# sarpel/wakeword-jupyterlab

Measured on AMD Instinct MI355X. Metric: 1s/16kHz clips/sec end-to-end (mel+CNN+LSTM), higher is better.
Workload: dtype f32 in/out/accumulate; conv and LSTM-gate GEMM products as f16x3 split (3 f16 MFMAs per fp32 product block, ~2^-21 rel.)

## Files before the change

### wakeword-jupyterlab_amd/csrc/ww_logmel.hip

```cpp
#include <mutex>
#include <type_traits>

#include "ww_internal.h"

namespace ww {

constexpr int kSlab = 2048 + 4;
constexpr int kPartialInSlab = 1032;
static_assert(kPartialInSlab + kPieces <= kSlab, "piece sums must fit behind the power spectrum");

template <int WAVES, int FR = kFrames>
struct K1Layout {
    static constexpr int kWaves = WAVES;
    static constexpr int kThreads = WAVES * 64;
    static constexpr int kMelStr = FR + 1;
    static constexpr int kOffMel = WAVES * kSlab;
    static constexpr int kOffRed = kOffMel + kMels * kMelStr;
    static constexpr int kOffFrm = kOffRed + 16;
    static constexpr int kOffInvw = kOffFrm + WAVES * FR;
    static constexpr int kOffFlag = kOffInvw + kMels;
    static constexpr int kOffDcNy = kOffFlag + 4;
    static constexpr int kOffPinfo = kOffDcNy + FR;
    static constexpr int kOffFp0 = kOffPinfo + kPieces;
    static constexpr int kOffFcnt = kOffFp0 + kMels;
    static constexpr int kOffTw2 = kOffFcnt + kMels;
    static constexpr int kOffTwp = kOffTw2 + 7 * 16 * 2;
    static constexpr int kLdsFloats = kOffTwp + 512 * 2;
    static constexpr int kWavesPerSimd = WAVES == 4 ? (FR != kFrames ? 2 : 3) : 2;
    static constexpr int kBlocksPerCu = WAVES == 4 ? (FR != kFrames ? 2 : 3) : 1;
    static_assert(kOffPinfo % 4 == 0 && kOffTw2 % 4 == 0 && kOffTwp % 2 == 0, "LDS table alignment");
    static_assert(FR % WAVES == 0 && WAVES <= 8, "frames are dealt to the waves in whole rounds; red[] holds 16 floats");
    static_assert(FR == kFrames || FR == 64, "the long-clip tile: 64 frames, frames dealt round-robin");
    static_assert(kBlocksPerCu * sizeof(float) * kLdsFloats <= 160 * 1024, "LDS per CU");
};

__device__ __forceinline__ float2 operator+(float2 a, float2 b) { return make_float2(a.x + b.x, a.y + b.y); }
__device__ __forceinline__ float2 operator-(float2 a, float2 b) { return make_float2(a.x - b.x, a.y - b.y); }
__device__ __forceinline__ float2 cmul(float2 a, float2 b) {
    return make_float2(fmaf(a.x, b.x, -a.y * b.y), fmaf(a.x, b.y, a.y * b.x));
}
__device__ __forceinline__ float2 mul_neg_i(float2 a) { return make_float2(a.y, -a.x); }

__device__ __forceinline__ void dft4(float2& a0, float2& a1, float2& a2, float2& a3) {
    const float2 t0 = a0 + a2, t1 = a0 - a2, t2 = a1 + a3, t3 = mul_neg_i(a1 - a3);
    a0 = t0 + t2; a2 = t0 - t2; a1 = t1 + t3; a3 = t1 - t3;
}

__device__ __forceinline__ void dft8(float2 (&v)[8]) {
    constexpr float c = 0.70710678118654752440f;
    float2 e0 = v[0], e1 = v[2], e2 = v[4], e3 = v[6];
    float2 o0 = v[1], o1 = v[3], o2 = v[5], o3 = v[7];
    dft4(e0, e1, e2, e3);
    dft4(o0, o1, o2, o3);
    o1 = make_float2(c * (o1.x + o1.y), c * (o1.y - o1.x));
    o2 = mul_neg_i(o2);
    o3 = make_float2(c * (o3.y - o3.x), -c * (o3.x + o3.y));
    v[0] = e0 + o0; v[4] = e0 - o0;
    v[1] = e1 + o1; v[5] = e1 - o1;
    v[2] = e2 + o2; v[6] = e2 - o2;
    v[3] = e3 + o3; v[7] = e3 - o3;
}

__device__ __forceinline__ void dft16(float2 (&v)[16]) {
    float2 e[8], o[8];
#pragma unroll
    for (int i = 0; i < 8; ++i) { e[i] = v[2 * i]; o[i] = v[2 * i + 1]; }
    dft8(e);
    dft8(o);
    constexpr float c1 = 0.92387953251128675613f, s1 = 0.38268343236508977173f;
    constexpr float c2 = 0.70710678118654752440f;
    const float2 w[8] = {{1.f, 0.f}, {c1, -s1}, {c2, -c2}, {s1, -c1}, {0.f, -1.f}, {-s1, -c1}, {-c2, -c2}, {-c1, -s1}};
#pragma unroll
    for (int k = 0; k < 8; ++k) {
        const float2 t = (k == 0) ? o[0] : (k == 4 ? mul_neg_i(o[4]) : cmul(o[k], w[k]));
        v[k] = e[k] + t;
        v[k + 8] = e[k] - t;
    }
}

__device__ __forceinline__ float db10(float x) {
#pragma clang fp contract(off)
    return 10.0f * log10f(x);
}

__device__ __forceinline__ void lds_order() {
    __builtin_amdgcn_fence(__ATOMIC_RELEASE, "wavefront");
    __builtin_amdgcn_wave_barrier();
    __builtin_amdgcn_fence(__ATOMIC_ACQUIRE, "wavefront");
}

__device__ __forceinline__ float absmax3(float a, float b, float m) {
    float r;
    asm("v_max3_f32 %0, |%1|, |%2|, %3" : "=v"(r) : "v"(a), "v"(b), "v"(m));
    return r;
}

using u32x4_t = __attribute__((ext_vector_type(4))) unsigned int;

template <bool RING>
__device__ __forceinline__ void load_frame(float4 (&sn)[8], __amdgpu_buffer_rsrc_t rsrc, int base, int ring_pos, int ring_len) {
#pragma unroll
    for (int n1 = 0; n1 < 8; ++n1) {
        const int idx = base + 256 * n1;
        int off = idx * 4;
        if constexpr (RING) {
            int at = idx + ring_pos;
            at = at >= ring_len ? at - ring_len : at;
            off = (idx >= 0 && idx < ring_len) ? at * 4 : -1;
        }
        const u32x4_t v = __builtin_amdgcn_raw_buffer_load_b128(rsrc, off, 0, 0);
        sn[n1] = __builtin_bit_cast(float4, v);
    }
}

constexpr uint32_t kRedoMark = 0x7fc5a11eu;
constexpr float kFloorRatio = 1.0e-5f;

#ifdef WW_STAMPS
__device__ unsigned long long g_stamps[16];
#define STAMP(i) do { unsigned long long t__; asm volatile("s_memtime %0\n\ts_waitcnt lgkmcnt(0)" : "=s"(t__) :: "memory"); \
    if (stamp_on) { acc_st[i] += t__ - last_st; } last_st = t__; } while (0)
#else
#define STAMP(i) do {} while (0)
#endif

template <bool RING, int WAVES, int FR = kFrames>
__global__ __launch_bounds__(WAVES * 64, (K1Layout<WAVES, FR>::kWavesPerSimd)) void logmel_kernel(const float* __restrict__ pcm, int64_t clip_stride,
                                                             int clip_len, int n_clips, int normalize,
                                                             const int32_t* __restrict__ ring_pos_p, int ring_len,
                                                             const LogmelTables* __restrict__ tb,
                                                             float* __restrict__ out, int mark, int n_frames) {
    using L = K1Layout<WAVES, FR>;
    constexpr int kMelStride = L::kMelStr;
    const int nfr = FR == kFrames ? kFrames : n_frames;
    constexpr int kWavesPerBlock = WAVES, kThreads = L::kThreads;
    constexpr int kOffMel = L::kOffMel, kOffRed = L::kOffRed, kOffFrm = L::kOffFrm, kOffInvw = L::kOffInvw, kOffFlag = L::kOffFlag,
                  kOffDcNy = L::kOffDcNy, kOffPinfo = L::kOffPinfo, kOffFp0 = L::kOffFp0,
                  kOffFcnt = L::kOffFcnt, kOffTw2 = L::kOffTw2, kOffTwp = L::kOffTwp;
    extern __shared__ __attribute__((aligned(16))) float lds[];
    float* mel = lds + kOffMel;
    float* red = lds + kOffRed;
    const float4* pw4 = reinterpret_cast<const float4*>(&tb->piece_w[0][0][0]);
    const int* pinfo = reinterpret_cast<const int*>(lds + kOffPinfo);
    const int* fp0 = reinterpret_cast<const int*>(lds + kOffFp0);
    const int* fcnt = reinterpret_cast<const int*>(lds + kOffFcnt);
    const float4* tw2_4 = reinterpret_cast<const float4*>(lds + kOffTw2);
    const float2* twp_2 = reinterpret_cast<const float2*>(lds + kOffTwp);

    const int tid = threadIdx.x;
    const int lane_id = tid & 63;
    const int lane = lane_id;
    const int wave = __builtin_amdgcn_readfirstlane(tid >> 6);
    float* slab = lds + wave * kSlab;
    float2* slab2 = reinterpret_cast<float2*>(slab);
    float4* slab4 = reinterpret_cast<float4*>(slab);
    float* partial = slab + kPartialInSlab;
    const float4* tw1_4 = reinterpret_cast<const float4*>(&tb->tw1[0][0]);
    const float4* win4 = reinterpret_cast<const float4*>(&tb->window[0]);

    for (int i = tid; i < kPieces; i += kThreads) reinterpret_cast<int*>(lds)[kOffPinfo + i] = tb->piece_info[i];
    if (tid < kMels) {
        reinterpret_cast<int*>(lds)[kOffFp0 + tid] = tb->filt_p0[tid];
        reinterpret_cast<int*>(lds)[kOffFcnt + tid] = tb->filt_cnt[tid];
        lds[kOffInvw + tid] = tb->band_bins[tid];
    }
    if (tid < 4) reinterpret_cast<uint32_t*>(lds)[kOffFlag + tid] = 0u;
    for (int i = tid; i < 7 * 16 * 2; i += kThreads) lds[kOffTw2 + i] = (&tb->tw2[0][0].x)[i];
    for (int i = tid; i < 512 * 2; i += kThreads) lds[kOffTwp + i] = (&tb->twp[0].x)[i];
    const int ring_pos = RING ? *ring_pos_p : 0;
    __syncthreads();
    const int my_p0a = fp0[lane], my_cnta = fcnt[lane];
    const int my_p0b = lane + 64 < kMels ? fp0[lane + 64] : 0, my_cntb = lane + 64 < kMels ? fcnt[lane + 64] : 0;

#ifdef WW_STAMPS
    const bool stamp_on = true;
    unsigned long long acc_st[10] = {0, 0, 0, 0, 0, 0, 0, 0, 0, 0}, last_st = 0;
    STAMP(9);
#endif

    const unsigned clip_bytes = unsigned(clip_len) * 4u;
    auto clip_rsrc = [&](int c) {
        const bool ok = c < n_clips;
        const float* base = pcm + int64_t(ok ? c : 0) * clip_stride;
        return __builtin_amdgcn_make_buffer_rsrc(const_cast<float*>(base), 0, ok ? clip_bytes : 0u, 0x00020000);
    };
    const int kRounds = FR == kFrames ? kFrames / kWavesPerBlock : (nfr + kWavesPerBlock - 1) / kWavesPerBlock;
    const int frame0 = wave;
    float4 sn[8];
    load_frame<RING>(sn, clip_rsrc(blockIdx.x), frame0 * kHop - kNfft / 2 + 4 * lane, ring_pos, ring_len);
    int clip_it = 0;
#pragma unroll 1
    for (int clip = blockIdx.x; clip < n_clips; clip += gridDim.x, ++clip_it) {
        const __amdgpu_buffer_rsrc_t rs_cur = clip_rsrc(clip), rs_next = clip_rsrc(clip + int(gridDim.x));
        float peak = 0.f;

#pragma unroll 1
        for (int round = 0; round < kRounds; ++round) {
            const int frame = round * kWavesPerBlock + wave;
            int lane = lane_id;
            asm volatile("" : "+v"(lane));
            const int k1r = lane >> 3, jr = lane & 7;
            const int base_next = (frame + kWavesPerBlock) * kHop - kNfft / 2 + 4 * lane;

            STAMP(8);
            float2 za[8], zb[8];
#pragma unroll
            for (int n1 = 0; n1 < 8; ++n1) {
                const float4 s = sn[n1];
                const float4 w = win4[64 * n1 + lane];
                if (n1 == 4 || n1 == 5) peak = absmax3(s.z, s.w, absmax3(s.x, s.y, peak));
                za[n1] = make_float2(s.x * w.x, s.y * w.y);
                zb[n1] = make_float2(s.z * w.z, s.w * w.w);
            }
            float4 t1[7];
#pragma unroll
            for (int k1 = 1; k1 < 8; ++k1) t1[k1 - 1] = tw1_4[(k1 - 1) * 64 + lane];
            __builtin_amdgcn_sched_barrier(0);
            dft8(za);
            dft8(zb);
            slab4[lane] = make_float4(za[0].x, za[0].y, zb[0].x, zb[0].y);
#pragma unroll
            for (int k1 = 1; k1 < 8; ++k1) {
                const float4 t = t1[k1 - 1];
                const float2 a = cmul(za[k1], make_float2(t.x, t.y));
                const float2 b = cmul(zb[k1], make_float2(t.z, t.w));
                slab4[k1 * 64 + (lane ^ (8 * ((k1 >> 1) & 1)))] = make_float4(a.x, a.y, b.x, b.y);
            }
            lds_order();
            STAMP(0);
            {
                const int s8 = 8 * ((k1r >> 1) & 1);
                const float4* x1e = slab4 + k1r * 64 + jr + s8;
                const float4* x1o = slab4 + k1r * 64 + jr - s8;
#pragma unroll
                for (int n2 = 0; n2 < 8; ++n2) {
                    const float4 v = (n2 & 1) ? x1o[n2 * 8] : x1e[n2 * 8];
                    za[n2] = make_float2(v.x, v.y);
                    zb[n2] = make_float2(v.z, v.w);
                }
                float4 t2[7];
#pragma unroll
                for (int k2 = 1; k2 < 8; ++k2) t2[k2 - 1] = tw2_4[(k2 - 1) * 8 + jr];
                lds_order();
                __builtin_amdgcn_sched_barrier(0);
                dft8(za);
                dft8(zb);
                float4* x2w[4];
#pragma unroll
                for (int hk = 0; hk < 4; ++hk) x2w[hk] = slab4 + 64 * k1r + (jr ^ (4 * (k1r & 1) + hk));
#pragma unroll
                for (int k2 = 0; k2 < 8; ++k2) {
                    float2 a = za[k2], b = zb[k2];
                    if (k2 > 0) {
                        const float4 t = t2[k2 - 1];
                        a = cmul(a, make_float2(t.x, t.y));
                        b = cmul(b, make_float2(t.z, t.w));
                    }
                    x2w[k2 >> 1][8 * k2] = make_float4(a.x, a.y, b.x, b.y);
                }
            }
            lds_order();
            STAMP(1);
            {
                float2 u[16];
                const int sw2 = (lane >> 1) & 7;
#pragma unroll
                for (int m = 0; m < 8; ++m) {
                    const float4 v = slab4[lane * 8 + (m ^ sw2)];
                    u[2 * m] = make_float2(v.x, v.y);
                    u[2 * m + 1] = make_float2(v.z, v.w);
                }
                lds_order();
                dft16(u);
                const int lp = (lane >> 3) + 8 * (lane & 7);
                float2* zw = slab2 + (lp ^ (((lp >> 4) & 3) << 1));
#pragma unroll
                for (int kk = 0; kk < 16; ++kk) zw[64 * kk] = u[kk];
            }
            lds_order();
            STAMP(2);
            float4 pw0[kPieceRounds], pw1[kPieceRounds];
#pragma unroll
            for (int c = 0; c < kPieceRounds; ++c) {
                pw0[c] = pw4[c * kPieceSlots + lane];
                pw1[c] = pw4[kPieces + c * kPieceSlots + lane];
            }
            {
                const bool last = round + 1 == kRounds;
                load_frame<RING>(sn, last ? rs_next : rs_cur, last ? frame0 * kHop - kNfft / 2 + 4 * lane : base_next, ring_pos,
                                 ring_len);
            }
            {
                float2 a[8], b[8];
                const int lowb = (64 - lane) & 63;
                const float2* za_p = slab2 + (lane ^ (((lane >> 4) & 3) << 1));
                const float2* zb_p = slab2 + (lowb ^ (((lowb >> 4) & 3) << 1)) + (lane == 0 ? 64 : 0);
#pragma unroll
                for (int j = 0; j < 8; ++j) {
                    a[j] = za_p[64 * j];
                    b[j] = zb_p[64 * (15 - j)];
                }
                if (lane == 0) {
                    if (mark) lds[kOffDcNy + frame] = 2.0f * fmaf(a[0].x, a[0].x, a[0].y * a[0].y);
                    a[0] = slab2[512];
                    b[0] = a[0];
                }
                float2 twj[8];
#pragma unroll
                for (int j = 0; j < 8; ++j) twj[j] = twp_2[lane + 64 * j];
                lds_order();
                __builtin_amdgcn_sched_barrier(0);
#pragma unroll
                for (int j = 0; j < 8; ++j) {
                    const int k = (j == 0 && lane == 0) ? 512 : lane + 64 * j;
                    const float2 tw = twj[j];
                    const float2 e = make_float2(0.5f * (a[j].x + b[j].x), 0.5f * (a[j].y - b[j].y));
                    const float2 o = make_float2(0.5f * (a[j].y + b[j].y), 0.5f * (b[j].x - a[j].x));
                    const float2 t = cmul(o, tw);
                    const float2 p = e + t, m = e - t;
                    slab[k] = fmaf(p.x, p.x, p.y * p.y);
                    slab[1024 - k] = fmaf(m.x, m.x, m.y * m.y);
                }
                if (lane == 0) slab[0] = 0.f;
            }
            lds_order();
            STAMP(3);
            {
                int info[kPieceRounds];
                float4 s0[kPieceRounds], s1[kPieceRounds];
#pragma unroll
                for (int c = 0; c < kPieceRounds; ++c) info[c] = pinfo[c * kPieceSlots + lane];
#pragma unroll
                for (int c = 0; c < kPieceRounds; ++c) {
                    const float4* s4 = reinterpret_cast<const float4*>(slab + (info[c] & 0xffff));
                    s0[c] = s4[0];
                    s1[c] = s4[1];
                }
                __builtin_amdgcn_sched_barrier(0);
#pragma unroll
                for (int c = 0; c < kPieceRounds; ++c) {
                    const float4 w0 = pw0[c], w1 = pw1[c];
                    float acc = w0.x * s0[c].x;
                    acc = fmaf(w0.y, s0[c].y, acc);
                    acc = fmaf(w0.z, s0[c].z, acc);
                    acc = fmaf(w0.w, s0[c].w, acc);
                    acc = fmaf(w1.x, s1[c].x, acc);
                    acc = fmaf(w1.y, s1[c].y, acc);
                    acc = fmaf(w1.z, s1[c].z, acc);
                    acc = fmaf(w1.w, s1[c].w, acc);
                    partial[info[c] >> 16] = acc;
                }
                lds_order();
                STAMP(4);
#pragma unroll
                for (int pass = 0; pass < 2; ++pass) {
                    const int f = lane + 64 * pass;
                    const int p0 = pass ? my_p0b : my_p0a, cnt = pass ? my_cntb : my_cnta;
                    if (f < kMels) {
                        float v[10];
#pragma unroll
                        for (int q = 0; q < 10; ++q) v[q] = partial[p0 + (q < cnt ? q : 0)];
                        float acc = 0.f;
#pragma unroll
                        for (int q = 0; q < 10; ++q) acc += (q < cnt) ? v[q] : 0.f;
                        mel[f * kMelStride + frame] = acc;
                    }
                }
            }
            lds_order();
            STAMP(5);
        }
        if constexpr (FR != kFrames) {
            __syncthreads();
            uint32_t* flag = reinterpret_cast<uint32_t*>(lds) + kOffFlag;
            if (mark && tid == 0) { flag[2 * ((clip_it + 1) & 1)] = 0u; flag[2 * ((clip_it + 1) & 1) + 1] = 0u; }
            const bool fr_live = lane < nfr;
            const float* invw = lds + kOffInvw;
            float* frm = lds + kOffFrm;
            float mmax = 0.f, e_part = 0.f;
            if (fr_live)
                for (int b = wave; b < kMels; b += kWavesPerBlock) {
                    const float p = mel[b * kMelStride + lane];
                    mmax = fmaxf(mmax, p);
                    if (mark) e_part = fmaf(p, invw[b], e_part);
                }
            if (mark) frm[wave * FR + lane] = e_part;
#pragma unroll
            for (int off = 32; off > 0; off >>= 1) {
                mmax = fmaxf(mmax, __shfl_xor(mmax, off));
                peak = fmaxf(peak, __shfl_xor(peak, off));
            }
            if (lane == 0) { red[wave] = mmax; red[kWavesPerBlock + wave] = peak; }
            __syncthreads();
            mmax = red[0];
            peak = red[kWavesPerBlock];
#pragma unroll
            for (int w = 1; w < kWavesPerBlock; ++w) { mmax = fmaxf(mmax, red[w]); peak = fmaxf(peak, red[kWavesPerBlock + w]); }
            const float amin = 1e-10f;
            float g2 = 1.f;
            if (normalize) { const float g = 1.0f / peak; g2 = g * g; }
            float ref = mmax * g2;
            ref = ref < amin ? amin : ref;
            const float ref_db = db10(ref);
            float* __restrict__ o = out + int64_t(clip) * (kMels * nfr);
            float floor_e = 0.f;
            if (mark) {
#pragma unroll
                for (int w = 0; w < kWavesPerBlock; ++w) floor_e += frm[w * FR + lane];
                floor_e += lds[kOffDcNy + lane];
                floor_e *= kFloorRatio;
            }
            const float live_thr = fmaxf(mmax * 0.99e-8f, amin / g2);
            bool redo = false;
            if (fr_live)
                for (int b = wave; b < kMels; b += kWavesPerBlock) {
                    const float p = mel[b * kMelStride + lane];
                    float v = p * g2;
                    v = v < amin ? amin : v;
                    float db = db10(v) - ref_db;
                    db = db < -80.0f ? -80.0f : db;
                    o[b * nfr + lane] = db;
                    if (mark) redo |= p > live_thr && p * invw[b] < floor_e;
                }
            if (mark) {
                const unsigned long long bal = __builtin_amdgcn_ballot_w64(redo);
                if (bal != 0ull && lane == 0) {
                    __hip_atomic_fetch_or(flag + 2 * (clip_it & 1), uint32_t(bal), __ATOMIC_RELAXED, __HIP_MEMORY_SCOPE_WORKGROUP);
                    __hip_atomic_fetch_or(flag + 2 * (clip_it & 1) + 1, uint32_t(bal >> 32), __ATOMIC_RELAXED, __HIP_MEMORY_SCOPE_WORKGROUP);
                }
            }
            __syncthreads();
            if (mark) {
                const uint32_t f_lo = flag[2 * (clip_it & 1)], f_hi = flag[2 * (clip_it & 1) + 1];
                if ((f_lo | f_hi) != 0u) {
                    if (fr_live)
                        for (int b = wave; b < kMels; b += kWavesPerBlock)
                            if (b * nfr + lane >= 3) o[b * nfr + lane] = mel[b * kMelStride + lane] * g2;
                    if (tid == 0) {
                        reinterpret_cast<uint32_t*>(o)[0] = kRedoMark;
                        reinterpret_cast<uint32_t*>(o)[1] = f_lo | 7u;
                        reinterpret_cast<uint32_t*>(o)[2] = f_hi;
                    }
                    __syncthreads();
                }
            }
        } else {
        __syncthreads();
        STAMP(6);
        uint32_t* flag = reinterpret_cast<uint32_t*>(lds) + kOffFlag;
        if (mark && tid == 0) flag[(clip_it + 1) & 1] = 0u;

        float mmax = 0.f, e_part = 0.f;
        const float* invw = lds + kOffInvw;
        float* frm = lds + kOffFrm;
        for (int idx = tid; idx < kMels * kFrames; idx += kThreads) {
            const float p = mel[(idx >> 5) * kMelStride + (idx & 31)];
            mmax = fmaxf(mmax, p);
            if (mark) e_part = fmaf(p, invw[idx >> 5], e_part);
        }
        if (mark) {
            e_part += __shfl_xor(e_part, 32);
            if (lane < 32) frm[wave * 32 + lane] = e_part;
        }
#pragma unroll
        for (int off = 32; off > 0; off >>= 1) {
            mmax = fmaxf(mmax, __shfl_xor(mmax, off));
            peak = fmaxf(peak, __shfl_xor(peak, off));
        }
        if (lane == 0) { red[wave] = mmax; red[kWavesPerBlock + wave] = peak; }
        __syncthreads();
        mmax = red[0];
        peak = red[kWavesPerBlock];
#pragma unroll
        for (int w = 1; w < kWavesPerBlock; ++w) { mmax = fmaxf(mmax, red[w]); peak = fmaxf(peak, red[kWavesPerBlock + w]); }

        const float amin = 1e-10f;
        float g2 = 1.f;
        if (normalize) { const float g = 1.0f / peak; g2 = g * g; }
        float ref = mmax * g2;
        ref = ref < amin ? amin : ref;
        const float ref_db = db10(ref);
        float* __restrict__ o = out + int64_t(clip) * (kMels * kFrames);
        float floor_e = 0.f;
        if (mark) {
#pragma unroll
            for (int w = 0; w < kWavesPerBlock; ++w) floor_e += frm[w * 32 + (tid & 31)];
            floor_e += lds[kOffDcNy + (tid & 31)];
            floor_e *= kFloorRatio;
        }
        const float live_thr = fmaxf(mmax * 0.99e-8f, amin / g2);
        bool redo = false;
        for (int idx = tid; idx < kMels * kFrames; idx += kThreads) {
            const float p = mel[(idx >> 5) * kMelStride + (idx & 31)];
            float v = p * g2;
            v = v < amin ? amin : v;
            float db = db10(v) - ref_db;
            db = db < -80.0f ? -80.0f : db;
            o[idx] = db;
            if (mark) redo |= p > live_thr && p * invw[idx >> 5] < floor_e;
        }
        if (mark) {
            const unsigned long long bal = __builtin_amdgcn_ballot_w64(redo);
            const uint32_t fm = uint32_t(bal) | uint32_t(bal >> 32);
            if (fm != 0u && lane == 0) __hip_atomic_fetch_or(flag + (clip_it & 1), fm, __ATOMIC_RELAXED, __HIP_MEMORY_SCOPE_WORKGROUP);
        }
        __syncthreads();
        if (mark) {
            const uint32_t fm = flag[clip_it & 1];
            if (fm != 0u) {
                for (int idx = tid; idx < kMels * kFrames; idx += kThreads)
                    if (idx >= 2) o[idx] = mel[(idx >> 5) * kMelStride + (idx & 31)] * g2;
                if (tid == 0) {
                    reinterpret_cast<uint32_t*>(o)[0] = kRedoMark;
                    reinterpret_cast<uint32_t*>(o)[1] = fm | 3u;
                }
            }
        }
        }
        STAMP(7);
    }
#ifdef WW_STAMPS
    if (lane == 0 && wave == 1 && blockIdx.x == 7)
        for (int i = 0; i < 10; ++i) atomicAdd(&g_stamps[i], acc_st[i]);
#endif
}
#ifdef WW_STAMPS
extern "C" __attribute__((visibility("default"))) int ww_debug_stamps(unsigned long long* out) {
    unsigned long long z[16] = {};
    if (hipMemcpyFromSymbol(out, HIP_SYMBOL(g_stamps), sizeof(z)) != hipSuccess) return -1;
    (void)hipMemcpyToSymbol(HIP_SYMBOL(g_stamps), z, sizeof(z));
    return 0;
}
#endif

struct cd { double x, y; };
struct alignas(16) cd2 { cd a, b; };
__device__ __forceinline__ cd operator+(cd a, cd b) { return {a.x + b.x, a.y + b.y}; }
__device__ __forceinline__ cd operator-(cd a, cd b) { return {a.x - b.x, a.y - b.y}; }
__device__ __forceinline__ cd cmul(cd a, cd b) { return {fma(a.x, b.x, -a.y * b.y), fma(a.x, b.y, a.y * b.x)}; }
__device__ __forceinline__ cd mul_neg_i(cd a) { return {a.y, -a.x}; }
__device__ __forceinline__ void dft4(cd& a0, cd& a1, cd& a2, cd& a3) {
    const cd t0 = a0 + a2, t1 = a0 - a2, t2 = a1 + a3, t3 = mul_neg_i(a1 - a3);
    a0 = t0 + t2; a2 = t0 - t2; a1 = t1 + t3; a3 = t1 - t3;
}
__device__ __forceinline__ void dft8(cd (&v)[8]) {
    constexpr double c = 0.70710678118654752440;
    cd e0 = v[0], e1 = v[2], e2 = v[4], e3 = v[6];
    cd o0 = v[1], o1 = v[3], o2 = v[5], o3 = v[7];
    dft4(e0, e1, e2, e3);
    dft4(o0, o1, o2, o3);
    o1 = {c * (o1.x + o1.y), c * (o1.y - o1.x)};
    o2 = mul_neg_i(o2);
    o3 = {c * (o3.y - o3.x), -c * (o3.x + o3.y)};
    v[0] = e0 + o0; v[4] = e0 - o0;
    v[1] = e1 + o1; v[5] = e1 - o1;
    v[2] = e2 + o2; v[6] = e2 - o2;
    v[3] = e3 + o3; v[7] = e3 - o3;
}
__device__ __forceinline__ void dft16(cd (&v)[16]) {
    cd e[8], o[8];
#pragma unroll
    for (int i = 0; i < 8; ++i) { e[i] = v[2 * i]; o[i] = v[2 * i + 1]; }
    dft8(e);
    dft8(o);
    constexpr double c1 = 0.92387953251128675613, s1 = 0.38268343236508977173, c2 = 0.70710678118654752440;
    const cd w[8] = {{1., 0.}, {c1, -s1}, {c2, -c2}, {s1, -c1}, {0., -1.}, {-s1, -c1}, {-c2, -c2}, {-c1, -s1}};
#pragma unroll
    for (int k = 0; k < 8; ++k) {
        const cd t = (k == 0) ? o[0] : (k == 4 ? mul_neg_i(o[4]) : cmul(o[k], w[k]));
        v[k] = e[k] + t;
        v[k + 8] = e[k] - t;
    }
}

constexpr int kSlab64 = 2 * 2048 + 8;
template <int FR = kFrames>
struct K64Layout {
    static constexpr int kMelStr = FR + 1;
    static constexpr int kOffMel = 4 * kSlab64;
    static constexpr int kOffRed = kOffMel + kMels * kMelStr;
    static constexpr int kOffPinfo = kOffRed + 16;
    static constexpr int kOffFp0 = kOffPinfo + kPieces;
    static constexpr int kOffFcnt = kOffFp0 + kMels;
    static constexpr int kOffTw2 = (kOffFcnt + kMels + 3) & ~3;
    static constexpr int kLdsFloats = kOffTw2 + 7 * 16 * 4;
    static constexpr int kBlocksPerCu = FR == kFrames ? 2 : 1;
    static_assert(kOffMel % 4 == 0 && kOffTw2 % 4 == 0, "16-byte alignment of the double tables");
    static_assert(kBlocksPerCu * (sizeof(float) * kLdsFloats + 512) <= 160 * 1024, "LDS per CU");
};
constexpr int k64LdsFloats = K64Layout<>::kLdsFloats;
static_assert(sizeof(float) * k64LdsFloats + 512 <= 80 * 1024, "two logmel64 workgroups per CU");

template <bool RING, bool ONLY_FLAGGED, int FR = kFrames>
__global__ __launch_bounds__(256, 2) void logmel64_kernel(const float* __restrict__ pcm, int64_t clip_stride, int clip_len, int n_clips,
                                                          int normalize, const int32_t* __restrict__ ring_pos_p, int ring_len,
                                                          const LogmelTables* __restrict__ tb, float* __restrict__ out, int n_frames) {
    constexpr int kWavesPerBlock = 4, kThreads = 256;
    using L64 = K64Layout<FR>;
    constexpr int kMelStride = L64::kMelStr, k64OffMel = L64::kOffMel, k64OffRed = L64::kOffRed, k64OffPinfo = L64::kOffPinfo,
                  k64OffFp0 = L64::kOffFp0, k64OffFcnt = L64::kOffFcnt, k64OffTw2 = L64::kOffTw2;
    const int nfr = FR == kFrames ? kFrames : n_frames;
    using mask_t = typename std::conditional<FR == kFrames, uint32_t, unsigned long long>::type;
    extern __shared__ __attribute__((aligned(16))) float lds[];
    float* mel = lds + k64OffMel;
    float* red = lds + k64OffRed;
    const int* pinfo = reinterpret_cast<const int*>(lds + k64OffPinfo);
    const int* fp0 = reinterpret_cast<const int*>(lds + k64OffFp0);
    const int* fcnt = reinterpret_cast<const int*>(lds + k64OffFcnt);
    const cd2* tw2_u = reinterpret_cast<const cd2*>(lds + k64OffTw2);
    const cd* twp_c = reinterpret_cast<const cd*>(&tb->twp_d[0]);
    const float4* pw4 = reinterpret_cast<const float4*>(&tb->piece_w[0][0][0]);
    const cd2* tw1_u = reinterpret_cast<const cd2*>(&tb->tw1_d[0][0]);
    const double* win = &tb->window_d[0];

    const int tid = threadIdx.x, lane_id = tid & 63, lane = lane_id;
    const int wave = __builtin_amdgcn_readfirstlane(tid >> 6);
    if constexpr (ONLY_FLAGGED) {
        int any = 0;
        for (int c = int(blockIdx.x) + tid * int(gridDim.x); c < n_clips; c += kThreads * int(gridDim.x))
            any |= __float_as_uint(__builtin_nontemporal_load(out + int64_t(c) * (kMels * nfr))) == kRedoMark;
        if (!__syncthreads_or(any)) return;
    }
    float* slabf = lds + wave * kSlab64;
    cd* slabc = reinterpret_cast<cd*>(slabf);
    cd* slabA = slabc;
    cd* slabB = slabc + 512;
    float* partial = slabf + kPartialInSlab;

    for (int i = tid; i < kPieces; i += kThreads) reinterpret_cast<int*>(lds)[k64OffPinfo + i] = tb->piece_info[i];
    if (tid < kMels) {
        reinterpret_cast<int*>(lds)[k64OffFp0 + tid] = tb->filt_p0[tid];
        reinterpret_cast<int*>(lds)[k64OffFcnt + tid] = tb->filt_cnt[tid];
    }
    for (int i = tid; i < 7 * 16 * 2; i += kThreads) reinterpret_cast<double*>(lds + k64OffTw2)[i] = (&tb->tw2_d[0][0].x)[i];
    const int ring_pos = RING ? *ring_pos_p : 0;
    __syncthreads();
    const int my_p0a = fp0[lane], my_cnta = fcnt[lane];
    const int my_p0b = lane + 64 < kMels ? fp0[lane + 64] : 0, my_cntb = lane + 64 < kMels ? fcnt[lane + 64] : 0;
    const unsigned clip_bytes = unsigned(clip_len) * 4u;

#pragma unroll 1
    for (int clip = blockIdx.x; clip < n_clips; clip += gridDim.x) {
        float* __restrict__ o = out + int64_t(clip) * (kMels * nfr);
        mask_t fmask = FR == kFrames ? mask_t(0xffffffffu) : (nfr >= 64 ? ~mask_t(0) : (mask_t(1) << nfr) - 1u);
        if constexpr (ONLY_FLAGGED) {
            if (__builtin_amdgcn_readfirstlane(__float_as_uint(__builtin_nontemporal_load(o))) != kRedoMark) continue;
            fmask = __builtin_amdgcn_readfirstlane(__float_as_uint(__builtin_nontemporal_load(o + 1)));
            if constexpr (FR != kFrames)
                fmask |= mask_t(__builtin_amdgcn_readfirstlane(__float_as_uint(__builtin_nontemporal_load(o + 2)))) << 32;
            for (int idx = tid; idx < kMels * nfr; idx += kThreads) {
                const int b = FR == kFrames ? idx >> 5 : idx / nfr, t = FR == kFrames ? idx & 31 : idx - b * nfr;
                if (!((fmask >> t) & 1u)) mel[b * kMelStride + t] = __builtin_nontemporal_load(o + idx);
            }
        }
        const int n_mine = (int(FR == kFrames ? __builtin_popcount(uint32_t(fmask)) : __builtin_popcountll(fmask)) - wave + kWavesPerBlock - 1) /
                           kWavesPerBlock;
        auto nth_frame = [&](int n) -> int {
            mask_t m = fmask;
            for (int i = 0; i < n && m; ++i) m &= m - 1u;
            return m ? (FR == kFrames ? __builtin_ctz(uint32_t(m)) : __builtin_ctzll(m)) : 2 * FR;
        };
        const __amdgpu_buffer_rsrc_t rs = __builtin_amdgcn_make_buffer_rsrc(const_cast<float*>(pcm + int64_t(clip) * clip_stride), 0,
                                                                             clip_bytes, 0x00020000);
        float peak = 0.f;
        if (normalize) {
#pragma unroll 1
            for (int round = 0; round < (nfr + kWavesPerBlock - 1) / kWavesPerBlock; ++round) {
                float4 sn[8];
                load_frame<RING>(sn, rs, (round * kWavesPerBlock + wave) * kHop - kNfft / 2 + 4 * lane, ring_pos, ring_len);
                peak = absmax3(sn[4].z, sn[4].w, absmax3(sn[4].x, sn[4].y, peak));
                peak = absmax3(sn[5].z, sn[5].w, absmax3(sn[5].x, sn[5].y, peak));
            }
#pragma unroll
            for (int off = 32; off > 0; off >>= 1) peak = fmaxf(peak, __shfl_xor(peak, off));
            if (lane == 0) red[wave] = peak;
            __syncthreads();
            peak = fmaxf(fmaxf(red[0], red[1]), fmaxf(red[2], red[3]));
            __syncthreads();
        }
        float4 sn[8];
        int frame = nth_frame(wave);
        load_frame<RING>(sn, rs, frame * kHop - kNfft / 2 + 4 * lane, ring_pos, ring_len);
#pragma unroll 1
        for (int round = 0; round < n_mine; ++round) {
            const int frame_next = nth_frame((round + 1) * kWavesPerBlock + wave);
            int lane = lane_id;
            asm volatile("" : "+v"(lane));
            const int k1r = lane >> 3, jr = lane & 7;
            cd za[8], zb[8];
#pragma unroll
            for (int n1 = 0; n1 < 8; ++n1) {
                float4 s = sn[n1];
                if (normalize) { s.x = __fdiv_rn(s.x, peak); s.y = __fdiv_rn(s.y, peak); s.z = __fdiv_rn(s.z, peak); s.w = __fdiv_rn(s.w, peak); }
                const double* w = win + 4 * (64 * n1 + lane);
                za[n1] = {double(s.x) * w[0], double(s.y) * w[1]};
                zb[n1] = {double(s.z) * w[2], double(s.w) * w[3]};
            }
            dft8(za);
            dft8(zb);
            slabA[lane] = za[0];
            slabB[lane] = zb[0];
#pragma unroll
            for (int k1 = 1; k1 < 8; ++k1) {
                const cd2 t = tw1_u[(k1 - 1) * 64 + lane];
                const int at = k1 * 64 + (lane ^ (8 * ((k1 >> 1) & 1)));
                slabA[at] = cmul(za[k1], t.a);
                slabB[at] = cmul(zb[k1], t.b);
            }
            lds_order();
            load_frame<RING>(sn, rs, frame_next * kHop - kNfft / 2 + 4 * lane, ring_pos, ring_len);
            {
                const int s8 = 8 * ((k1r >> 1) & 1);
                const cd* x1e = slabA + k1r * 64 + jr + s8;
                const cd* x1o = slabA + k1r * 64 + jr - s8;
#pragma unroll
                for (int n2 = 0; n2 < 8; ++n2) {
                    const cd* src = (n2 & 1) ? x1o + n2 * 8 : x1e + n2 * 8;
                    za[n2] = src[0];
                    zb[n2] = src[512];
                }
                lds_order();
                dft8(za);
                dft8(zb);
                cd* x2w[4];
#pragma unroll
                for (int hk = 0; hk < 4; ++hk) x2w[hk] = slabA + 64 * k1r + (jr ^ (4 * (k1r & 1) + hk));
#pragma unroll
                for (int k2 = 0; k2 < 8; ++k2) {
                    cd a = za[k2], b = zb[k2];
                    if (k2 > 0) {
                        const cd2 t = tw2_u[(k2 - 1) * 8 + jr];
                        a = cmul(a, t.a);
                        b = cmul(b, t.b);
                    }
                    x2w[k2 >> 1][8 * k2] = a;
                    x2w[k2 >> 1][8 * k2 + 512] = b;
                }
            }
            lds_order();
            {
                cd u[16];
                const int sw2 = (lane >> 1) & 7;
#pragma unroll
                for (int m = 0; m < 8; ++m) {
                    const cd* src = slabA + lane * 8 + (m ^ sw2);
                    u[2 * m] = src[0];
                    u[2 * m + 1] = src[512];
                }
                lds_order();
                dft16(u);
                const int lp = (lane >> 3) + 8 * (lane & 7);
                cd* zw = slabc + (lp ^ ((lp >> 3) & 7));
#pragma unroll
                for (int kk = 0; kk < 16; ++kk) zw[64 * kk] = u[kk];
            }
            lds_order();
            {
                cd a[8], b[8];
                const int lowb = (64 - lane) & 63;
                const cd* za_p = slabc + (lane ^ ((lane >> 3) & 7));
                const cd* zb_p = slabc + (lowb ^ ((lowb >> 3) & 7)) + (lane == 0 ? 64 : 0);
#pragma unroll
                for (int j = 0; j < 8; ++j) {
                    a[j] = za_p[64 * j];
                    b[j] = zb_p[64 * (15 - j)];
                }
                if (lane == 0) { a[0] = slabc[512]; b[0] = a[0]; }
                lds_order();
#pragma unroll
                for (int j = 0; j < 8; ++j) {
                    const int k = (j == 0 && lane == 0) ? 512 : lane + 64 * j;
                    const cd tw = twp_c[lane + 64 * j];
                    const cd e = {0.5 * (a[j].x + b[j].x), 0.5 * (a[j].y - b[j].y)};
                    const cd od = {0.5 * (a[j].y + b[j].y), 0.5 * (b[j].x - a[j].x)};
                    const cd t = cmul(od, tw);
                    const float px = float(e.x + t.x), py = float(e.y + t.y), mx = float(e.x - t.x), my = float(e.y - t.y);
                    slabf[k] = fmaf(px, px, py * py);
                    slabf[1024 - k] = fmaf(mx, mx, my * my);
                }
                if (lane == 0) slabf[0] = 0.f;
            }
            lds_order();
            {
                int info[kPieceRounds];
                float4 s0[kPieceRounds], s1[kPieceRounds], pw0[kPieceRounds], pw1[kPieceRounds];
#pragma unroll
                for (int c = 0; c < kPieceRounds; ++c) {
                    info[c] = pinfo[c * kPieceSlots + lane];
                    pw0[c] = pw4[c * kPieceSlots + lane];
                    pw1[c] = pw4[kPieces + c * kPieceSlots + lane];
                }
#pragma unroll
                for (int c = 0; c < kPieceRounds; ++c) {
                    const float4* s4 = reinterpret_cast<const float4*>(slabf + (info[c] & 0xffff));
                    s0[c] = s4[0];
                    s1[c] = s4[1];
                }
#pragma unroll
                for (int c = 0; c < kPieceRounds; ++c) {
                    const float4 w0 = pw0[c], w1 = pw1[c];
                    float acc = w0.x * s0[c].x;
                    acc = fmaf(w0.y, s0[c].y, acc);
                    acc = fmaf(w0.z, s0[c].z, acc);
                    acc = fmaf(w0.w, s0[c].w, acc);
                    acc = fmaf(w1.x, s1[c].x, acc);
                    acc = fmaf(w1.y, s1[c].y, acc);
                    acc = fmaf(w1.z, s1[c].z, acc);
                    acc = fmaf(w1.w, s1[c].w, acc);
                    partial[info[c] >> 16] = acc;
                }
                lds_order();
#pragma unroll
                for (int pass = 0; pass < 2; ++pass) {
                    const int f = lane + 64 * pass;
                    const int p0 = pass ? my_p0b : my_p0a, cnt = pass ? my_cntb : my_cnta;
                    if (f < kMels) {
                        float acc = 0.f;
                        for (int q = 0; q < cnt; ++q) acc += partial[p0 + q];
                        mel[f * kMelStride + frame] = acc;
                    }
                }
            }
            lds_order();
            frame = frame_next;
        }
        __syncthreads();
        float mmax = 0.f;
        bool any_nan = false;
        for (int idx = tid; idx < kMels * nfr; idx += kThreads) {
            const int b = FR == kFrames ? idx >> 5 : idx / nfr, t = FR == kFrames ? idx & 31 : idx - b * nfr;
            const float p = mel[b * kMelStride + t];
            any_nan |= p != p;
            mmax = fmaxf(mmax, p);
        }
#pragma unroll
        for (int off = 32; off > 0; off >>= 1) mmax = fmaxf(mmax, __shfl_xor(mmax, off));
        any_nan = __builtin_amdgcn_ballot_w64(any_nan) != 0ull;
        if (lane == 0) red[wave] = any_nan ? __uint_as_float(0x7fc00000u) : mmax;
        __syncthreads();
        mmax = red[0];
#pragma unroll
        for (int w = 1; w < kWavesPerBlock; ++w) mmax = (red[w] != red[w] || mmax != mmax) ? __uint_as_float(0x7fc00000u) : fmaxf(mmax, red[w]);
        const float amin = 1e-10f;
        float ref = mmax;
        ref = ref < amin ? amin : ref;
        const float ref_db = db10(ref);
        for (int idx = tid; idx < kMels * nfr; idx += kThreads) {
            const int b = FR == kFrames ? idx >> 5 : idx / nfr, t = FR == kFrames ? idx & 31 : idx - b * nfr;
            float v = mel[b * kMelStride + t];
            v = v < amin ? amin : v;
            float db = db10(v) - ref_db;
            db = db < -80.0f ? -80.0f : db;
            o[idx] = db;
        }
        __syncthreads();
    }
}

template <int WAVES, int FR = kFrames>
static int launch_logmel_w(const float* pcm, int64_t n_clips, int64_t clip_stride, int64_t clip_len, int normalize,
                           const int32_t* ring_pos, int64_t ring_len, float* logmel, const LogmelTables* tb, int mark, hipStream_t stream,
                           int n_frames = kFrames) {
    using L = K1Layout<WAVES, FR>;
    const int64_t resident = int64_t(device_cu_count()) * L::kBlocksPerCu;
    const int grid = int(n_clips < resident ? n_clips : resident);
    const size_t lds_bytes = sizeof(float) * L::kLdsFloats;
    if (ring_pos)
        hipLaunchKernelGGL((logmel_kernel<true, WAVES, FR>), dim3(grid), dim3(L::kThreads), lds_bytes, stream, pcm, clip_stride, int(clip_len),
                           int(n_clips), normalize, ring_pos, int(ring_len), tb, logmel, mark, n_frames);
    else
        hipLaunchKernelGGL((logmel_kernel<false, WAVES, FR>), dim3(grid), dim3(L::kThreads), lds_bytes, stream, pcm, clip_stride, int(clip_len),
                           int(n_clips), normalize, ring_pos, int(ring_len), tb, logmel, mark, n_frames);
    WW_HIP(hipGetLastError());
    return WW_OK;
}

template <bool ONLY_FLAGGED, int FR = kFrames>
static int launch_logmel64(const float* pcm, int64_t n_clips, int64_t clip_stride, int64_t clip_len, int normalize,
                           const int32_t* ring_pos, int64_t ring_len, float* logmel, const LogmelTables* tb, hipStream_t stream,
                           int n_frames = kFrames) {
    const int64_t resident = K64Layout<FR>::kBlocksPerCu * int64_t(device_cu_count());
    const int grid = int(n_clips < resident ? n_clips : resident);
    const size_t lds_bytes = sizeof(float) * K64Layout<FR>::kLdsFloats;
    if (ring_pos)
        hipLaunchKernelGGL((logmel64_kernel<true, ONLY_FLAGGED, FR>), dim3(grid), dim3(256), lds_bytes, stream, pcm, clip_stride, int(clip_len),
                           int(n_clips), normalize, ring_pos, int(ring_len), tb, logmel, n_frames);
    else
        hipLaunchKernelGGL((logmel64_kernel<false, ONLY_FLAGGED, FR>), dim3(grid), dim3(256), lds_bytes, stream, pcm, clip_stride, int(clip_len),
                           int(n_clips), normalize, ring_pos, int(ring_len), tb, logmel, n_frames);
    WW_HIP(hipGetLastError());
    return WW_OK;
}

static int logmel_opt_in_lds() {
    static std::mutex mu;
    static bool done[64] = {};
    std::lock_guard<std::mutex> lock(mu);
    int dev = 0;
    WW_HIP(hipGetDevice(&dev));
    if (dev < 0 || dev >= 64) return fail(WW_EINVAL, "device ordinal out of range");
    if (done[dev]) return WW_OK;
    const int b4 = int(sizeof(float) * K1Layout<4>::kLdsFloats), b8 = int(sizeof(float) * K1Layout<8>::kLdsFloats);
    const int b64 = int(sizeof(float) * k64LdsFloats);
    WW_HIP(hipFuncSetAttribute(reinterpret_cast<const void*>(logmel_kernel<true, 4>), hipFuncAttributeMaxDynamicSharedMemorySize, b4));
    WW_HIP(hipFuncSetAttribute(reinterpret_cast<const void*>(logmel_kernel<false, 4>), hipFuncAttributeMaxDynamicSharedMemorySize, b4));
    WW_HIP(hipFuncSetAttribute(reinterpret_cast<const void*>(logmel_kernel<true, 8>), hipFuncAttributeMaxDynamicSharedMemorySize, b8));
    WW_HIP(hipFuncSetAttribute(reinterpret_cast<const void*>(logmel_kernel<false, 8>), hipFuncAttributeMaxDynamicSharedMemorySize, b8));
    WW_HIP(hipFuncSetAttribute(reinterpret_cast<const void*>(logmel64_kernel<true, true>), hipFuncAttributeMaxDynamicSharedMemorySize, b64));
    WW_HIP(hipFuncSetAttribute(reinterpret_cast<const void*>(logmel64_kernel<true, false>), hipFuncAttributeMaxDynamicSharedMemorySize, b64));
    WW_HIP(hipFuncSetAttribute(reinterpret_cast<const void*>(logmel64_kernel<false, true>), hipFuncAttributeMaxDynamicSharedMemorySize, b64));
    WW_HIP(hipFuncSetAttribute(reinterpret_cast<const void*>(logmel64_kernel<false, false>), hipFuncAttributeMaxDynamicSharedMemorySize, b64));
    const int c4 = int(sizeof(float) * K1Layout<4, 64>::kLdsFloats), c8 = int(sizeof(float) * K1Layout<8, 64>::kLdsFloats);
    const int c64 = int(sizeof(float) * K64Layout<64>::kLdsFloats);
    WW_HIP(hipFuncSetAttribute(reinterpret_cast<const void*>(logmel_kernel<true, 4, 64>), hipFuncAttributeMaxDynamicSharedMemorySize, c4));
    WW_HIP(hipFuncSetAttribute(reinterpret_cast<const void*>(logmel_kernel<false, 4, 64>), hipFuncAttributeMaxDynamicSharedMemorySize, c4));
    WW_HIP(hipFuncSetAttribute(reinterpret_cast<const void*>(logmel_kernel<true, 8, 64>), hipFuncAttributeMaxDynamicSharedMemorySize, c8));
    WW_HIP(hipFuncSetAttribute(reinterpret_cast<const void*>(logmel_kernel<false, 8, 64>), hipFuncAttributeMaxDynamicSharedMemorySize, c8));
    WW_HIP(hipFuncSetAttribute(reinterpret_cast<const void*>(logmel64_kernel<true, true, 64>), hipFuncAttributeMaxDynamicSharedMemorySize, c64));
    WW_HIP(hipFuncSetAttribute(reinterpret_cast<const void*>(logmel64_kernel<true, false, 64>), hipFuncAttributeMaxDynamicSharedMemorySize, c64));
    WW_HIP(hipFuncSetAttribute(reinterpret_cast<const void*>(logmel64_kernel<false, true, 64>), hipFuncAttributeMaxDynamicSharedMemorySize, c64));
    WW_HIP(hipFuncSetAttribute(reinterpret_cast<const void*>(logmel64_kernel<false, false, 64>), hipFuncAttributeMaxDynamicSharedMemorySize, c64));
    done[dev] = true;
    return WW_OK;
}

int launch_logmel(const float* pcm, int64_t n_clips, int64_t clip_stride, int64_t clip_len, int normalize,
                  const int32_t* ring_pos, int64_t ring_len, float* logmel, hipStream_t stream) {
    if (n_clips == 0) return WW_OK;
    const LogmelTables* tb = device_tables();
    if (!tb) return WW_EHIP;
    if (int rc = logmel_opt_in_lds()) return rc;
    const int mode = logmel_math_mode();
    if (mode == WW_LOGMEL_MATH_F64)
        return launch_logmel64<false>(pcm, n_clips, clip_stride, clip_len, normalize, ring_pos, ring_len, logmel, tb, stream);
    const int mark = mode == WW_LOGMEL_MATH_AUTO;
    int rc;
    if (n_clips <= device_cu_count())
        rc = launch_logmel_w<8>(pcm, n_clips, clip_stride, clip_len, normalize, ring_pos, ring_len, logmel, tb, mark, stream);
    else
        rc = launch_logmel_w<4>(pcm, n_clips, clip_stride, clip_len, normalize, ring_pos, ring_len, logmel, tb, mark, stream);
    if (rc != WW_OK || !mark) return rc;
    return launch_logmel64<true>(pcm, n_clips, clip_stride, clip_len, normalize, ring_pos, ring_len, logmel, tb, stream);
}

int launch_logmel_frames(const float* pcm, int64_t n_clips, int64_t clip_stride, int64_t clip_len, int64_t n_samples, int normalize,
                         const int32_t* ring_pos, int64_t ring_len, float* logmel, hipStream_t stream) {
    const int T = int(1 + n_samples / kHop);
    if (T == kFrames) return launch_logmel(pcm, n_clips, clip_stride, clip_len, normalize, ring_pos, ring_len, logmel, stream);
    if (n_clips == 0) return WW_OK;
    const LogmelTables* tb = device_tables();
    if (!tb) return WW_EHIP;
    if (int rc = logmel_opt_in_lds()) return rc;
    const int mode = logmel_math_mode();
    if (mode == WW_LOGMEL_MATH_F64)
        return launch_logmel64<false, 64>(pcm, n_clips, clip_stride, clip_len, normalize, ring_pos, ring_len, logmel, tb, stream, T);
    const int mark = mode == WW_LOGMEL_MATH_AUTO;
    int rc;
    if (n_clips <= device_cu_count())
        rc = launch_logmel_w<8, 64>(pcm, n_clips, clip_stride, clip_len, normalize, ring_pos, ring_len, logmel, tb, mark, stream, T);
    else
        rc = launch_logmel_w<4, 64>(pcm, n_clips, clip_stride, clip_len, normalize, ring_pos, ring_len, logmel, tb, mark, stream, T);
    if (rc != WW_OK || !mark) return rc;
    return launch_logmel64<true, 64>(pcm, n_clips, clip_stride, clip_len, normalize, ring_pos, ring_len, logmel, tb, stream, T);
}
int launch_logmel_frames(const float* pcm, int64_t n_clips, int64_t clip_stride, int64_t clip_len, int64_t n_samples, int normalize,
                         float* logmel, hipStream_t stream) {
    return launch_logmel_frames(pcm, n_clips, clip_stride, clip_len, n_samples, normalize, nullptr, 0, logmel, stream);
}

}
```

Before: 4.845 million.

## Record flagged clips in a device redo list and early-hand-off hopeless clips to f64

The fp32 logmel kernel now appends each clip it marks for redo to a per-stream device list via an atomic counter. The f64 fix-up kernel reads that list and processes only the listed clips, replacing its scan of every clip's output header. It also adds an early exit after the first round: if every wave's first frame already fails the precision-floor test, the block marks the whole clip for f64 redo and skips the remaining fp32 rounds. In exchange it adds per-stream device allocation and host bookkeeping, a block barrier in round zero, and atomic counter reset logic that must hold across launches.

```diff
diff --git a/wakeword-jupyterlab_amd/csrc/ww_logmel.hip b/wakeword-jupyterlab_amd/csrc/ww_logmel.hip
--- a/wakeword-jupyterlab_amd/csrc/ww_logmel.hip
+++ b/wakeword-jupyterlab_amd/csrc/ww_logmel.hip
@@ -1,5 +1,7 @@
 #include <mutex>
+#include <thread>
 #include <type_traits>
+#include <vector>
 
 #include "ww_internal.h"
 
@@ -116,6 +118,14 @@
 constexpr uint32_t kRedoMark = 0x7fc5a11eu;
 constexpr float kFloorRatio = 1.0e-5f;
 
+constexpr int kRedoHdr = 8, kRedoCap = 8192, kRedoWords = kRedoHdr + kRedoCap, kRedoRecords = 32;
+
+__device__ __forceinline__ void redo_append(uint32_t* rec, int clip) {
+    if (!rec) return;
+    const uint32_t slot = __hip_atomic_fetch_add(rec, 1u, __ATOMIC_RELAXED, __HIP_MEMORY_SCOPE_AGENT);
+    if (slot < uint32_t(kRedoCap)) rec[kRedoHdr + slot] = uint32_t(clip);
+}
+
 #ifdef WW_STAMPS
 __device__ unsigned long long g_stamps[16];
 #define STAMP(i) do { unsigned long long t__; asm volatile("s_memtime %0\n\ts_waitcnt lgkmcnt(0)" : "=s"(t__) :: "memory"); \
@@ -129,7 +139,8 @@
                                                              int clip_len, int n_clips, int normalize,
                                                              const int32_t* __restrict__ ring_pos_p, int ring_len,
                                                              const LogmelTables* __restrict__ tb,
-                                                             float* __restrict__ out, int mark, int n_frames) {
+                                                             float* __restrict__ out, int mark, int n_frames,
+                                                             uint32_t* __restrict__ redo_rec) {
     using L = K1Layout<WAVES, FR>;
     constexpr int kMelStride = L::kMelStr;
     const int nfr = FR == kFrames ? kFrames : n_frames;
@@ -193,6 +204,7 @@
     for (int clip = blockIdx.x; clip < n_clips; clip += gridDim.x, ++clip_it) {
         const __amdgpu_buffer_rsrc_t rs_cur = clip_rsrc(clip), rs_next = clip_rsrc(clip + int(gridDim.x));
         float peak = 0.f;
+        bool handed_over = false;
 
 #pragma unroll 1
         for (int round = 0; round < kRounds; ++round) {
@@ -369,6 +381,55 @@
             }
             lds_order();
             STAMP(5);
+            if (mark && round == 0) {
+                const float* invw = lds + kOffInvw;
+                const bool two = lane + 64 < kMels;
+                const float pa = mel[lane * kMelStride + frame], wa = invw[lane];
+                const float pb = two ? mel[(lane + 64) * kMelStride + frame] : 0.f, wb = two ? invw[lane + 64] : 0.f;
+                float e = fmaf(pb, wb, pa * wa), fmx = fmaxf(pa, pb), pk = peak;
+#pragma unroll
+                for (int off = 32; off > 0; off >>= 1) {
+                    e += __shfl_xor(e, off);
+                    fmx = fmaxf(fmx, __shfl_xor(fmx, off));
+                    pk = fmaxf(pk, __shfl_xor(pk, off));
+                }
+                float g2 = 1.f;
+                if (normalize) { const float g = 1.0f / pk; g2 = g * g; }
+                const float thr = fmaxf(fmx * 0.99e-8f, 1e-10f / g2);
+                const float floor_e = (e + lds[kOffDcNy + frame]) * kFloorRatio;
+                const bool hit = (pa > thr && pa * wa < floor_e) || (pb > thr && pb * wb < floor_e);
+                float* vote = red + (clip_it & 1) * kWavesPerBlock;
+                if (lane == 0) vote[wave] = __builtin_amdgcn_ballot_w64(hit) != 0ull ? 1.f : 0.f;
+                __syncthreads();
+                bool all = true;
+#pragma unroll
+                for (int w = 0; w < kWavesPerBlock; ++w) all = all && vote[w] != 0.f;
+                if (all) {
+                    if (round + 1 != kRounds)
+                        load_frame<RING>(sn, rs_next, frame0 * kHop - kNfft / 2 + 4 * lane, ring_pos, ring_len);
+                    handed_over = true;
+                    break;
+                }
+            }
+        }
+        if (handed_over) {
+            if (tid == 0) {
+                uint32_t* o = reinterpret_cast<uint32_t*>(out + int64_t(clip) * (kMels * nfr));
+                uint32_t* flag = reinterpret_cast<uint32_t*>(lds) + kOffFlag;
+                o[0] = kRedoMark;
+                if constexpr (FR == kFrames) {
+                    o[1] = 0xffffffffu;
+                    flag[(clip_it + 1) & 1] = 0u;
+                } else {
+                    const unsigned long long full = nfr >= 64 ? ~0ull : (1ull << nfr) - 1ull;
+                    o[1] = uint32_t(full);
+                    o[2] = uint32_t(full >> 32);
+                    flag[2 * ((clip_it + 1) & 1)] = 0u;
+                    flag[2 * ((clip_it + 1) & 1) + 1] = 0u;
+                }
+                redo_append(redo_rec, clip);
+            }
+            continue;
         }
         if constexpr (FR != kFrames) {
             __syncthreads();
@@ -440,6 +501,7 @@
                         reinterpret_cast<uint32_t*>(o)[0] = kRedoMark;
                         reinterpret_cast<uint32_t*>(o)[1] = f_lo | 7u;
                         reinterpret_cast<uint32_t*>(o)[2] = f_hi;
+                        redo_append(redo_rec, clip);
                     }
                     __syncthreads();
                 }
@@ -513,7 +575,9 @@
                 if (tid == 0) {
                     reinterpret_cast<uint32_t*>(o)[0] = kRedoMark;
                     reinterpret_cast<uint32_t*>(o)[1] = fm | 3u;
-                }
+                    redo_append(redo_rec, clip);
+                }
+                __syncthreads();
             }
         }
         }
@@ -594,7 +658,8 @@
 template <bool RING, bool ONLY_FLAGGED, int FR = kFrames>
 __global__ __launch_bounds__(256, 2) void logmel64_kernel(const float* __restrict__ pcm, int64_t clip_stride, int clip_len, int n_clips,
                                                           int normalize, const int32_t* __restrict__ ring_pos_p, int ring_len,
-                                                          const LogmelTables* __restrict__ tb, float* __restrict__ out, int n_frames) {
+                                                          const LogmelTables* __restrict__ tb, float* __restrict__ out, int n_frames,
+                                                          uint32_t* __restrict__ redo_rec) {
     constexpr int kWavesPerBlock = 4, kThreads = 256;
     using L64 = K64Layout<FR>;
     constexpr int kMelStride = L64::kMelStr, k64OffMel = L64::kOffMel, k64OffRed = L64::kOffRed, k64OffPinfo = L64::kOffPinfo,
@@ -615,11 +680,32 @@
 
     const int tid = threadIdx.x, lane_id = tid & 63, lane = lane_id;
     const int wave = __builtin_amdgcn_readfirstlane(tid >> 6);
+    int n_work = n_clips;
+    bool listed = false;
     if constexpr (ONLY_FLAGGED) {
-        int any = 0;
-        for (int c = int(blockIdx.x) + tid * int(gridDim.x); c < n_clips; c += kThreads * int(gridDim.x))
-            any |= __float_as_uint(__builtin_nontemporal_load(out + int64_t(c) * (kMels * nfr))) == kRedoMark;
-        if (!__syncthreads_or(any)) return;
+        if (redo_rec) {
+            uint32_t* red_u = reinterpret_cast<uint32_t*>(red);
+            if (tid == 0) {
+                const uint32_t cnt = __hip_atomic_load(redo_rec, __ATOMIC_RELAXED, __HIP_MEMORY_SCOPE_AGENT);
+                red_u[0] = cnt;
+                const uint32_t seen = __hip_atomic_fetch_add(redo_rec + 1, 1u, __ATOMIC_RELEASE, __HIP_MEMORY_SCOPE_AGENT);
+                if (seen + 1u == gridDim.x) {
+                    __hip_atomic_store(redo_rec, 0u, __ATOMIC_RELAXED, __HIP_MEMORY_SCOPE_AGENT);
+                    __hip_atomic_store(redo_rec + 1, 0u, __ATOMIC_RELAXED, __HIP_MEMORY_SCOPE_AGENT);
+                }
+            }
+            __syncthreads();
+            const uint32_t cnt = red_u[0];
+            if (cnt == 0u) return;
+            __syncthreads();
+            listed = cnt <= uint32_t(kRedoCap);
+            if (listed) n_work = int(cnt);
+        } else {
+            int any = 0;
+            for (int c = int(blockIdx.x) + tid * int(gridDim.x); c < n_clips; c += kThreads * int(gridDim.x))
+                any |= __float_as_uint(__builtin_nontemporal_load(out + int64_t(c) * (kMels * nfr))) == kRedoMark;
+            if (!__syncthreads_or(any)) return;
+        }
     }
     float* slabf = lds + wave * kSlab64;
     cd* slabc = reinterpret_cast<cd*>(slabf);
@@ -640,7 +726,14 @@
     const unsigned clip_bytes = unsigned(clip_len) * 4u;
 
 #pragma unroll 1
-    for (int clip = blockIdx.x; clip < n_clips; clip += gridDim.x) {
+    for (int work = blockIdx.x; work < n_work; work += gridDim.x) {
+        int clip = work;
+        if constexpr (ONLY_FLAGGED) {
+            if (listed) {
+                clip = __builtin_amdgcn_readfirstlane(int(redo_rec[kRedoHdr + work]));
+                if (unsigned(clip) >= unsigned(n_clips)) continue;
+            }
+        }
         float* __restrict__ o = out + int64_t(clip) * (kMels * nfr);
         mask_t fmask = FR == kFrames ? mask_t(0xffffffffu) : (nfr >= 64 ? ~mask_t(0) : (mask_t(1) << nfr) - 1u);
         if constexpr (ONLY_FLAGGED) {
@@ -860,17 +953,17 @@
 template <int WAVES, int FR = kFrames>
 static int launch_logmel_w(const float* pcm, int64_t n_clips, int64_t clip_stride, int64_t clip_len, int normalize,
                            const int32_t* ring_pos, int64_t ring_len, float* logmel, const LogmelTables* tb, int mark, hipStream_t stream,
-                           int n_frames = kFrames) {
+                           uint32_t* redo_rec, int n_frames = kFrames) {
     using L = K1Layout<WAVES, FR>;
     const int64_t resident = int64_t(device_cu_count()) * L::kBlocksPerCu;
     const int grid = int(n_clips < resident ? n_clips : resident);
     const size_t lds_bytes = sizeof(float) * L::kLdsFloats;
     if (ring_pos)
         hipLaunchKernelGGL((logmel_kernel<true, WAVES, FR>), dim3(grid), dim3(L::kThreads), lds_bytes, stream, pcm, clip_stride, int(clip_len),
-                           int(n_clips), normalize, ring_pos, int(ring_len), tb, logmel, mark, n_frames);
+                           int(n_clips), normalize, ring_pos, int(ring_len), tb, logmel, mark, n_frames, redo_rec);
     else
         hipLaunchKernelGGL((logmel_kernel<false, WAVES, FR>), dim3(grid), dim3(L::kThreads), lds_bytes, stream, pcm, clip_stride, int(clip_len),
-                           int(n_clips), normalize, ring_pos, int(ring_len), tb, logmel, mark, n_frames);
+                           int(n_clips), normalize, ring_pos, int(ring_len), tb, logmel, mark, n_frames, redo_rec);
     WW_HIP(hipGetLastError());
     return WW_OK;
 }
@@ -878,16 +971,16 @@
 template <bool ONLY_FLAGGED, int FR = kFrames>
 static int launch_logmel64(const float* pcm, int64_t n_clips, int64_t clip_stride, int64_t clip_len, int normalize,
                            const int32_t* ring_pos, int64_t ring_len, float* logmel, const LogmelTables* tb, hipStream_t stream,
-                           int n_frames = kFrames) {
+                           uint32_t* redo_rec, int n_frames = kFrames) {
     const int64_t resident = K64Layout<FR>::kBlocksPerCu * int64_t(device_cu_count());
     const int grid = int(n_clips < resident ? n_clips : resident);
     const size_t lds_bytes = sizeof(float) * K64Layout<FR>::kLdsFloats;
     if (ring_pos)
         hipLaunchKernelGGL((logmel64_kernel<true, ONLY_FLAGGED, FR>), dim3(grid), dim3(256), lds_bytes, stream, pcm, clip_stride, int(clip_len),
-                           int(n_clips), normalize, ring_pos, int(ring_len), tb, logmel, n_frames);
+                           int(n_clips), normalize, ring_pos, int(ring_len), tb, logmel, n_frames, redo_rec);
     else
         hipLaunchKernelGGL((logmel64_kernel<false, ONLY_FLAGGED, FR>), dim3(grid), dim3(256), lds_bytes, stream, pcm, clip_stride, int(clip_len),
-                           int(n_clips), normalize, ring_pos, int(ring_len), tb, logmel, n_frames);
+                           int(n_clips), normalize, ring_pos, int(ring_len), tb, logmel, n_frames, redo_rec);
     WW_HIP(hipGetLastError());
     return WW_OK;
 }
@@ -924,6 +1017,43 @@
     return WW_OK;
 }
 
+static uint32_t* redo_record(hipStream_t stream) {
+    struct Key { int dev; hipStream_t stream; std::thread::id thread; };
+    static std::mutex mu;
+    static uint32_t* slab[64] = {};
+    static std::vector<Key> keys;
+    static int used[64] = {};
+    int dev = 0;
+    if (hipGetDevice(&dev) != hipSuccess || dev < 0 || dev >= 64) return nullptr;
+    hipStreamCaptureStatus cap = hipStreamCaptureStatusNone;
+    if (hipStreamIsCapturing(stream, &cap) != hipSuccess || cap != hipStreamCaptureStatusNone) {
+        (void)hipGetLastError();
+        return nullptr;
+    }
+    const Key key{dev, stream, stream == hipStreamPerThread ? std::this_thread::get_id() : std::thread::id()};
+    std::lock_guard<std::mutex> lock(mu);
+    if (!slab[dev]) {
+        uint32_t* p = nullptr;
+        const size_t bytes = sizeof(uint32_t) * kRedoWords * kRedoRecords;
+        if (hipMalloc(reinterpret_cast<void**>(&p), bytes) != hipSuccess || hipMemset(p, 0, bytes) != hipSuccess ||
+            hipDeviceSynchronize() != hipSuccess) {
+            (void)hipGetLastError();
+            if (p) (void)hipFree(p);
+            return nullptr;
+        }
+        slab[dev] = p;
+    }
+    int index = 0;
+    for (const Key& k : keys) {
+        if (k.dev != dev) continue;
+        if (k.stream == stream && k.thread == key.thread) return slab[dev] + size_t(index) * kRedoWords;
+        ++index;
+    }
+    if (used[dev] >= kRedoRecords) return nullptr;
+    keys.push_back(key);
+    return slab[dev] + size_t(used[dev]++) * kRedoWords;
+}
+
 int launch_logmel(const float* pcm, int64_t n_clips, int64_t clip_stride, int64_t clip_len, int normalize,
                   const int32_t* ring_pos, int64_t ring_len, float* logmel, hipStream_t stream) {
     if (n_clips == 0) return WW_OK;
@@ -932,15 +1062,16 @@
     if (int rc = logmel_opt_in_lds()) return rc;
     const int mode = logmel_math_mode();
     if (mode == WW_LOGMEL_MATH_F64)
-        return launch_logmel64<false>(pcm, n_clips, clip_stride, clip_len, normalize, ring_pos, ring_len, logmel, tb, stream);
+        return launch_logmel64<false>(pcm, n_clips, clip_stride, clip_len, normalize, ring_pos, ring_len, logmel, tb, stream, nullptr);
     const int mark = mode == WW_LOGMEL_MATH_AUTO;
+    uint32_t* rec = mark ? redo_record(stream) : nullptr;
     int rc;
     if (n_clips <= device_cu_count())
-        rc = launch_logmel_w<8>(pcm, n_clips, clip_stride, clip_len, normalize, ring_pos, ring_len, logmel, tb, mark, stream);
+        rc = launch_logmel_w<8>(pcm, n_clips, clip_stride, clip_len, normalize, ring_pos, ring_len, logmel, tb, mark, stream, rec);
     else
-        rc = launch_logmel_w<4>(pcm, n_clips, clip_stride, clip_len, normalize, ring_pos, ring_len, logmel, tb, mark, stream);
+        rc = launch_logmel_w<4>(pcm, n_clips, clip_stride, clip_len, normalize, ring_pos, ring_len, logmel, tb, mark, stream, rec);
     if (rc != WW_OK || !mark) return rc;
-    return launch_logmel64<true>(pcm, n_clips, clip_stride, clip_len, normalize, ring_pos, ring_len, logmel, tb, stream);
+    return launch_logmel64<true>(pcm, n_clips, clip_stride, clip_len, normalize, ring_pos, ring_len, logmel, tb, stream, rec);
 }
 
 int launch_logmel_frames(const float* pcm, int64_t n_clips, int64_t clip_stride, int64_t clip_len, int64_t n_samples, int normalize,
@@ -953,15 +1084,16 @@
     if (int rc = logmel_opt_in_lds()) return rc;
     const int mode = logmel_math_mode();
     if (mode == WW_LOGMEL_MATH_F64)
-        return launch_logmel64<false, 64>(pcm, n_clips, clip_stride, clip_len, normalize, ring_pos, ring_len, logmel, tb, stream, T);
+        return launch_logmel64<false, 64>(pcm, n_clips, clip_stride, clip_len, normalize, ring_pos, ring_len, logmel, tb, stream, nullptr, T);
     const int mark = mode == WW_LOGMEL_MATH_AUTO;
+    uint32_t* rec = mark ? redo_record(stream) : nullptr;
     int rc;
     if (n_clips <= device_cu_count())
-        rc = launch_logmel_w<8, 64>(pcm, n_clips, clip_stride, clip_len, normalize, ring_pos, ring_len, logmel, tb, mark, stream, T);
+        rc = launch_logmel_w<8, 64>(pcm, n_clips, clip_stride, clip_len, normalize, ring_pos, ring_len, logmel, tb, mark, stream, rec, T);
     else
-        rc = launch_logmel_w<4, 64>(pcm, n_clips, clip_stride, clip_len, normalize, ring_pos, ring_len, logmel, tb, mark, stream, T);
+        rc = launch_logmel_w<4, 64>(pcm, n_clips, clip_stride, clip_len, normalize, ring_pos, ring_len, logmel, tb, mark, stream, rec, T);
     if (rc != WW_OK || !mark) return rc;
-    return launch_logmel64<true, 64>(pcm, n_clips, clip_stride, clip_len, normalize, ring_pos, ring_len, logmel, tb, stream, T);
+    return launch_logmel64<true, 64>(pcm, n_clips, clip_stride, clip_len, normalize, ring_pos, ring_len, logmel, tb, stream, rec, T);
 }
 int launch_logmel_frames(const float* pcm, int64_t n_clips, int64_t clip_stride, int64_t clip_len, int64_t n_samples, int normalize,
                          float* logmel, hipStream_t stream) {
```

New measurement: 4.795 million. 0.99x the previous value.
